# MaciejKozarzewski/AlphaGomoku

Hardware: AMD Instinct MI355X
Metric: MCTS simulations/sec (self-play, 15x15 freestyle) (higher is better)
Workload: dtype f16 (network, fp32 accumulate) + int/fp32 (tree)

## Files before the change

alphagomoku_amd/csrc/nn_forward.hip:

```cpp
#include "agx_internal.hpp"
#include "nn_any_board.hpp"

#include <vector>
#include <mutex>
#include <utility>
#include <cstring>
#include <cmath>
#include <cstdlib>
#include <type_traits>

#ifndef AGX_NN_COLS_AHEAD
#define AGX_NN_COLS_AHEAD 4
#endif
#ifndef AGX_NN_COLS_PAD
#define AGX_NN_COLS_PAD 1
#endif
#ifndef AGX_NN_ROW_GROUPS
#define AGX_NN_ROW_GROUPS 8
#endif
#ifndef AGX_NN_PAIR_BALANCE
#define AGX_NN_PAIR_BALANCE 1
#endif
#ifndef AGX_NN_AHEAD
#define AGX_NN_AHEAD 4
#endif

namespace
{
	typedef _Float16 half_t;
	typedef _Float16 half8 __attribute__((ext_vector_type(8)));
	typedef _Float16 half4 __attribute__((ext_vector_type(4)));
	typedef _Float16 half2 __attribute__((ext_vector_type(2)));
	typedef float floatx4 __attribute__((ext_vector_type(4)));

	struct NetParams
	{
			const half8 *w_in;
			const half8 *w_tower;
			const float *bias;
			const float *wp2;
			const float *wv1;
			const half_t *wv2;
			half_t *vhead_x;
			const float *bv2;
			const float *wv3;
			float bp2;
			float bv1[4];
			float bv3[3];
			int blocks;
			int batch;
			const int *slot_list;
			const int *count_ptr;
			const float *wq2;
			float bq2[3];
			float *q;
			half4 *skip;
	};

#ifdef AGX_NN_PROFILE
	__device__ unsigned long long g_nn_prof[2][16];
	struct NnStamp
	{
			unsigned long long last;
			bool on;
			int row;
			__device__ NnStamp(int wave, int lane) :
					last(clock64()), on(lane == 0 && (wave & 3) == 0), row(wave >> 2)
			{
			}
			__device__ void mark(int k)
			{
				const unsigned long long now = clock64();
				if (on)
					atomicAdd(&g_nn_prof[row][k], now - last);
				last = now;
			}
	};
#define AGX_NN_MARK(K) stamp.mark(K)
#define AGX_NN_STAMP_PARAM , NnStamp &stamp
#define AGX_NN_STAMP_ARG , stamp
#else
#define AGX_NN_MARK(K) do { } while (0)
#define AGX_NN_STAMP_PARAM
#define AGX_NN_STAMP_ARG
#endif

	template<int F, int ROWS, int COLS>
	struct Geometry
	{
			static constexpr int S = COLS + 1;
			static constexpr int NT = (ROWS * S + 15) / 16;
			static constexpr int NPOS = 1 + S + NT * 16 + S + 2;
			static constexpr int CH = F / 8;
			static constexpr int PPR = (16 / CH) > 0 ? (16 / CH) : 1;
			static constexpr bool COLT = (ROWS == 20 && COLS == 20 && F == 128);
			static constexpr int CG = (S == 16 && F >= 128) ? AGX_NN_ROW_GROUPS : ((S == 16 || F >= 128) ? 4 : 2);
			static constexpr int PG = 8 / CG;
			static constexpr int MT = F / (16 * CG);
			static constexpr int WRING = 2;
			static constexpr int STAGE_TAPS = 3;
			static constexpr int COL_TILES = COLS / PG, TAIL_TILES = 6 / PG, TAIL_FIRST = 21;
			static constexpr int PAD = COLT ? AGX_NN_COLS_PAD : 0;
			static constexpr int POS_BYTES = F * 2 + 16 * PAD;
			static constexpr int PLANE_BYTES = NPOS * POS_BYTES;
			static constexpr int NTW = COLT ? (COL_TILES + TAIL_TILES) : (NT + PG - 1) / PG;
			static constexpr int THREADS = 512;
			__device__ static __forceinline__ int channel_group(int wave) { return wave & (CG - 1); }
			__device__ static __forceinline__ int first_tile(int wave) { return (wave >> (CG == 8 ? 3 : (CG == 4 ? 2 : 1))) * NTW; }
			__device__ static __forceinline__ int swizzle(int index)
			{
				if constexpr (PAD > 0)
					return 0;
				else
					return (index / PPR) % CH;
			}
			__device__ static __forceinline__ int slot(int index, int chunk) { return chunk ^ swizzle(index); }
			__device__ static __forceinline__ int tile_position(int wave, int n, int r)
			{
				if constexpr (COLT)
				{
					const int pg = wave >> (CG == 8 ? 3 : 2);
					return (n < COL_TILES) ? (r * S + pg * COL_TILES + n) : ((TAIL_FIRST + pg * TAIL_TILES + (n - COL_TILES)) * 16 + r);
				}
				else
					return (first_tile(wave) + n) * 16 + r;
			}
			__device__ static __forceinline__ int tile_count(int wave)
			{
				if constexpr (COLT)
					return NTW;
				else if constexpr (PG == 1)
					return NT;
				else if constexpr (PG == 2)
					return (wave >> 2) ? (NT - NTW) : NTW;
				else
					return ((wave >> 1) == PG - 1) ? (NT - (PG - 1) * NTW) : NTW;
			}
			static constexpr int MTILES = F / 16;
			static constexpr int KC = F / 32;
			static constexpr int S5 = (S == 16 && F >= 128) ? 32 : S + 4;
			static constexpr int NPOS5 = (ROWS + 4) * S5 + 4;
			static constexpr int HW = ROWS * COLS;
			static constexpr int D = (2 * F < 256) ? 2 * F : 256;
			static constexpr int KPAD = (HW * 4 + 31) / 32 * 32;
			static constexpr int SCRATCH_FLOATS = HW * 4 + D + 8 + 256 + 8 + F * 4 + F + F * 4;
			static constexpr int LDS_BYTES = 2 * PLANE_BYTES + SCRATCH_FLOATS * 4;
			static constexpr int LDS_BYTES_INPLACE = PLANE_BYTES + SCRATCH_FLOATS * 4 + CG * NT * 16 * 4 + 3 * NT * 16 * 4;
			static constexpr int SKIP_PER_WG = 8 * MT * NTW * 64;
	};

	__device__ __forceinline__ void lds_barrier()
	{
		__builtin_amdgcn_fence(__ATOMIC_RELEASE, "workgroup", "local");
		__builtin_amdgcn_s_barrier();
		__builtin_amdgcn_fence(__ATOMIC_ACQUIRE, "workgroup", "local");
	}
	__device__ __forceinline__ int* pair_progress()
	{
		__shared__ int progress[8];
		return progress;
	}
	struct PairBalance
	{
			typedef __attribute__((address_space(3))) int lds_int;
			volatile lds_int *mine;
			const volatile lds_int *partner;
			int tick, seen;
			__device__ __forceinline__ PairBalance(int *progress, int wave) :
					mine((volatile lds_int*) (progress + wave)), partner((const volatile lds_int*) (progress + (wave ^ 4))), tick(progress[wave]), seen(progress[wave ^ 4])
			{
			}
			__device__ __forceinline__ void turn()
			{
#if AGX_NN_PAIR_BALANCE
				const int ahead = __builtin_amdgcn_readfirstlane(tick - seen);
				if (ahead > 0)
					__builtin_amdgcn_s_setprio(1);
				else if (ahead == 0)
					__builtin_amdgcn_s_setprio(2);
				else
					__builtin_amdgcn_s_setprio(3);
#endif
			}
			__device__ __forceinline__ void done()
			{
#if AGX_NN_PAIR_BALANCE
				tick++;
				*mine = tick;
				seen = *partner;
#endif
			}
	};
	template<typename G>
	__device__ __forceinline__ int plane_offset(int index, int chunk)
	{
		return index * G::POS_BYTES + G::slot(index, chunk) * 16;
// ... 924 lines not shown
						b[u] = fragment(u + 1);
#pragma unroll
					for (int j = 1; j <= G::NTW + 1; j++)
					{
						const int jn = j + AHEAD - 1;
						if (jn <= G::NTW + 1)
							b[(jn - 1) % AHEAD] = fragment(jn);
#pragma unroll
						for (int dyi = 3; dyi < 5; dyi++)
						{
							const int o = j - (dyi - 2);
							if (o >= 0 && o < G::NTW && o < my_tiles)
							{
#pragma unroll
								for (int i = 0; i < G::MT; i++)
									acc[i][o] = __builtin_amdgcn_mfma_f32_16x16x32_f16(a_down[dyi - 3][i], b[(j - 1) % AHEAD], acc[i][o], 0, 0, 0);
							}
						}
						__builtin_amdgcn_sched_barrier(0);
					}
				}
			}
		}
		else
		{
			int q0[G::NTW];
	#pragma unroll
			for (int n = 0; n < G::NTW; n++)
			{
				const int pos = G::S + G::tile_position(wave, n, r);
				const int x = pos % G::S;
				const int y = pos / G::S - 1;
				q0[n] = (y + 2) * G::S5 + (x + 2);
			}

			const half8 *wp = wpk + (mg * G::MT) * 64 + lane;
			half8 a_next[G::MT];
	#pragma unroll
			for (int i = 0; i < G::MT; i++)
				a_next[i] = wp[i * 64];
	#pragma unroll 1
			for (int t = 0; t < 25; t++)
			{
				const int off = (t / 5 - 2) * G::S5 + (t % 5 - 2);
				half8 a[G::MT];
	#pragma unroll
				for (int i = 0; i < G::MT; i++)
					a[i] = a_next[i];
				const int tn = (t + 1 < 25) ? (t + 1) : 0;
	#pragma unroll
				for (int i = 0; i < G::MT; i++)
					a_next[i] = wp[(tn * G::MTILES + i) * 64];
	#pragma unroll
				for (int n = 0; n < G::NTW; n++)
					if (n < my_tiles)
					{
						int q = q0[n] + off;
						q = (q < 0) ? 0 : ((q >= G::NPOS5) ? (G::NPOS5 - 1) : q);
						const half8 b = *reinterpret_cast<const half8*>(in5 + (q * 4 + (q4 ^ ((q >> 2) & 3))) * 16);
	#pragma unroll
						for (int i = 0; i < G::MT; i++)
							acc[i][n] = __builtin_amdgcn_mfma_f32_16x16x32_f16(a[i], b, acc[i][n], 0, 0, 0);
					}
			}
		}
		if (INPLACE)
		{
			__syncthreads();
			const uint4 zero4 = make_uint4(0u, 0u, 0u, 0u);
			for (int i = wave * 64 + lane; i < G::PLANE_BYTES / 16; i += G::THREADS)
				reinterpret_cast<uint4*>(dst)[i] = zero4;
			__syncthreads();
		}
		typedef __attribute__((address_space(1))) half4 global_half4;
		int skip_lane = lane;
		asm volatile("" : "+v"(skip_lane));
		global_half4 *my_skip = (global_half4*) (skip + __builtin_amdgcn_readfirstlane(wave * G::MT * G::NTW * 64)) + skip_lane;
		if constexpr (G::S == 16 && !INPLACE)
		{
			static_assert(G::NT == ROWS, "a tile is a board row + the spare column");
			if (r < COLS)
			{
#pragma unroll
				for (int i = 0; i < G::MT; i++)
				{
					const int ch = (mg * G::MT + i) * 16 + 4 * q4;
					const floatx4 bv = *reinterpret_cast<const floatx4*>(bias + ch);
					char *out0 = dst + plane_offset<G>(1 + G::S + n0 * 16 + r, ch / 8) + (ch % 8) * 2;
#pragma unroll
					for (int n = 0; n < G::NTW; n++)
						if (n < my_tiles)
						{
							const floatx4 v = acc[i][n];
							half2 lo { static_cast<half_t>(v[0] + bv[0]), static_cast<half_t>(v[1] + bv[1]) }, hi { static_cast<half_t>(v[2] + bv[2]), static_cast<half_t>(v[3] + bv[3]) };
							const half2 zero2 { static_cast<half_t>(0.0f), static_cast<half_t>(0.0f) };
							lo = __builtin_elementwise_max(lo, zero2);
							hi = __builtin_elementwise_max(hi, zero2);
							*reinterpret_cast<uint2*>(out0 + n * 16 * G::POS_BYTES) = uint2 { __builtin_bit_cast(uint32_t, lo), __builtin_bit_cast(uint32_t, hi) };
						}
				}
			}
			return;
		}
#pragma unroll
		for (int i = 0; i < G::MT; i++)
		{
			const int ch = (mg * G::MT + i) * 16 + 4 * q4;
			const floatx4 bv = *reinterpret_cast<const floatx4*>(bias + ch);
#pragma unroll
			for (int n = 0; n < G::NTW; n++)
				if (n < my_tiles)
				{
					const int pos = G::S + G::tile_position(wave, n, r);
					const int x = pos % G::S;
					const int y = pos / G::S - 1;
					const bool valid = (x < COLS) && (y < ROWS);
					char *ptr = dst + plane_offset<G>(pos + 1, ch / 8) + (ch % 8) * 2;
					const floatx4 v = acc[i][n] + bv;
					half4 o;
					o[0] = static_cast<half_t>(valid ? fmaxf(v[0], 0.0f) : 0.0f);
					o[1] = static_cast<half_t>(valid ? fmaxf(v[1], 0.0f) : 0.0f);
					o[2] = static_cast<half_t>(valid ? fmaxf(v[2], 0.0f) : 0.0f);
					o[3] = static_cast<half_t>(valid ? fmaxf(v[3], 0.0f) : 0.0f);
					*reinterpret_cast<half4*>(ptr) = o;
					if (INPLACE)
						my_skip[(i * G::NTW + n) * 64] = o;
				}
		}
	}

	__device__ __forceinline__ float block_reduce_max(float v, float *red, int tid)
	{
#pragma unroll
		for (int o = 32; o > 0; o >>= 1)
			v = fmaxf(v, __shfl_xor(v, o));
		__syncthreads();
		if ((tid & 63) == 0)
			red[tid >> 6] = v;
		__syncthreads();
		return fmaxf(fmaxf(fmaxf(red[0], red[1]), fmaxf(red[2], red[3])), fmaxf(fmaxf(red[4], red[5]), fmaxf(red[6], red[7])));
	}
	__device__ __forceinline__ float block_reduce_sum(float v, float *red, int tid)
	{
#pragma unroll
		for (int o = 32; o > 0; o >>= 1)
			v += __shfl_xor(v, o);
		__syncthreads();
		if ((tid & 63) == 0)
			red[tid >> 6] = v;
		__syncthreads();
		return ((red[0] + red[1]) + (red[2] + red[3])) + ((red[4] + red[5]) + (red[6] + red[7]));
	}

	template<int F, int ROWS, int COLS, bool INPLACE, bool QHEAD, bool RAW = false>
#ifndef AGX_NN_WAVES_PER_EU
#define AGX_NN_WAVES_PER_EU 2
#endif
	__global__ __launch_bounds__(256 * AGX_NN_WAVES_PER_EU) void nn_tower_kernel(NetParams p, const uint32_t *__restrict__ features, float *__restrict__ policy,
			float *__restrict__ value)
	{
		typedef Geometry<F, ROWS, COLS> G;
		constexpr int LDS_TOTAL = INPLACE ? G::LDS_BYTES_INPLACE : G::LDS_BYTES;
		static_assert(LDS_TOTAL <= 163840, "board does not fit in LDS");
		static_assert(G::NPOS5 * 64 <= G::PLANE_BYTES, "padded input plane must fit into an activation plane");
		__shared__ __attribute__((aligned(16))) char lds[LDS_TOTAL];
		char *plane_x = lds;
		char *plane_t = INPLACE ? lds : lds + G::PLANE_BYTES;
		float *vbuf = reinterpret_cast<float*>(lds + (INPLACE ? 1 : 2) * G::PLANE_BYTES);
		half8 *s_wv1f = reinterpret_cast<half8*>(vbuf);
		static_assert(G::KC * 64 * 16 <= (G::HW * 4 + G::D) * 4, "value-head fragments must fit into the former vbuf + hid area");
		float *hid = vbuf + G::HW * 4;
		float *red = hid + G::D;
		float *s_wv1 = red + 8 + 256 + 8;
		float *s_wp2 = s_wv1 + F * 4;
		float *s_wq2 = s_wp2 + F;
		float *ppart = s_wq2 + F * 4;
		float *qpart = ppart + G::CG * G::NT * 16;
		half4 *skip = INPLACE ? (p.skip + static_cast<size_t>(blockIdx.x) * G::SKIP_PER_WG) : nullptr;

		const int tid = threadIdx.x;
		const int wave = tid >> 6;
		const int lane = tid & 63;
		const int layer_halves8 = 9 * G::KC * G::MTILES * 64;

		const uint4 zero4 = make_uint4(0u, 0u, 0u, 0u);
		for (int i = tid; i < G::PLANE_BYTES / 16; i += G::THREADS)
			reinterpret_cast<uint4*>(plane_x)[i] = zero4;
		for (int i = tid; i < G::KC * 64; i += G::THREADS)
		{
			const int kc = i / 64, l = i % 64, unit = l & 15;
			half8 f;
#pragma unroll
			for (int j = 0; j < 8; j++)
				f[j] = static_cast<half_t>((unit < 4) ? p.wv1[(kc * 32 + 8 * (l >> 4) + j) * 4 + unit] : 0.0f);
			s_wv1f[i] = f;
		}
		for (int i = tid; i < F; i += G::THREADS)
			s_wp2[i] = p.wp2[i];
		if (QHEAD)
			for (int i = tid; i < F * 4; i += G::THREADS)
				s_wq2[i] = p.wq2[i];

#if AGX_NN_PAIR_BALANCE
		if (tid < 8)
			pair_progress()[tid] = 0;
#endif
		const int batch = (p.count_ptr != nullptr) ? min(*p.count_ptr, p.batch) : p.batch;
#ifdef AGX_NN_PROFILE
		NnStamp stamp(wave, lane);
#endif
		static_assert(G::HW <= G::THREADS, "one feature word per thread");
		uint32_t next_word = 0;
		if (static_cast<int>(blockIdx.x) < batch && tid < G::HW)
			next_word = features[static_cast<size_t>((p.slot_list != nullptr) ? p.slot_list[blockIdx.x] : static_cast<int>(blockIdx.x)) * G::HW + tid];
		for (int bi = blockIdx.x; bi < batch; bi += gridDim.x)
		{
			const int b = (p.slot_list != nullptr) ? p.slot_list[bi] : bi;
			__syncthreads();
			for (int i = tid; i < G::NPOS5 * (RAW ? 1 : 4); i += G::THREADS)
				reinterpret_cast<uint4*>(plane_t)[i] = zero4;
			__syncthreads();
			for (int c = tid; c < G::HW; c += G::THREADS)
			{
				const uint32_t word = next_word;
				const int q = (c / COLS + 2) * G::S5 + (c % COLS + 2);
#pragma unroll
				for (int k = 0; k < (RAW ? 1 : 4); k++)
				{
					const uint32_t bits = (word >> (8 * k)) & 255u;
					uint4 v;
					v.x = ((bits & 1u) ? 0x3C00u : 0u) | ((bits & 2u) ? 0x3C000000u : 0u);
					v.y = ((bits & 4u) ? 0x3C00u : 0u) | ((bits & 8u) ? 0x3C000000u : 0u);
					v.z = ((bits & 16u) ? 0x3C00u : 0u) | ((bits & 32u) ? 0x3C000000u : 0u);
					v.w = ((bits & 64u) ? 0x3C00u : 0u) | ((bits & 128u) ? 0x3C000000u : 0u);
					if (RAW)
						*reinterpret_cast<uint4*>(plane_t + q * 16) = v;
					else
						*reinterpret_cast<uint4*>(plane_t + (q * 4 + (k ^ ((q >> 2) & 3))) * 16) = v;
				}
			}
			__syncthreads();
			AGX_NN_MARK(0);
			conv5x5_input<F, ROWS, COLS, INPLACE, RAW>(plane_t, plane_x, p.w_in, p.bias, skip, wave, lane);
			BiasCarry<G::MT> bias_carry;
			request_bias<G>(p.bias + F, wave, lane, bias_carry);
			__syncthreads();
			AGX_NN_MARK(1);
			if (!INPLACE)
			{
				for (int i = tid; i < G::PLANE_BYTES / 16; i += G::THREADS)
					reinterpret_cast<uint4*>(plane_t)[i] = zero4;
				__syncthreads();
			}

			AGX_NN_MARK(9);
			constexpr bool CARRY = INPLACE ? (G::COLT && !RAW) : G::S == 16;
			WeightCarry<G> carry_store;
			WeightCarry<G> *carry = CARRY ? &carry_store : nullptr;
			if constexpr (CARRY)
				request_first_stage<F, ROWS, COLS>(p.w_tower, wave, lane, carry_store);
			for (int blk = 0; blk < p.blocks; blk++)
			{
				if (INPLACE)
				{
					SkipCarry<G> skip_carry;
					if constexpr (CARRY)
						carry_store.next = p.w_tower + (2 * blk + 1) * layer_halves8;
					conv3x3_inplace<F, ROWS, COLS, 0>(plane_x, p.w_tower + (2 * blk) * layer_halves8, bias_carry, p.bias + (2 + 2 * blk) * F, skip, nullptr, nullptr, wave,
							lane AGX_NN_STAMP_ARG, &skip_carry, carry);
					lds_barrier();
					if constexpr (CARRY)
						carry_store.next = p.w_tower + (2 * blk + 2) * layer_halves8;
					conv3x3_inplace<F, ROWS, COLS, 1>(plane_x, p.w_tower + (2 * blk + 1) * layer_halves8, bias_carry, p.bias + (3 + 2 * blk) * F, skip, nullptr, nullptr, wave,
							lane AGX_NN_STAMP_ARG, &skip_carry, carry);
					lds_barrier();
				}
				else
				{
					if constexpr (CARRY)
						carry_store.next = p.w_tower + (2 * blk + 1) * layer_halves8;
					conv3x3<F, ROWS, COLS, false>(plane_x, plane_t, p.w_tower + (2 * blk) * layer_halves8, p.bias + (1 + 2 * blk) * F, wave, lane AGX_NN_STAMP_ARG, carry, &bias_carry,
							p.bias + (2 + 2 * blk) * F);
					__syncthreads();
					AGX_NN_MARK(5);
					if constexpr (CARRY)
						carry_store.next = p.w_tower + (2 * blk + 2) * layer_halves8;
					conv3x3<F, ROWS, COLS, true>(plane_t, plane_x, p.w_tower + (2 * blk + 1) * layer_halves8, p.bias + (2 + 2 * blk) * F, wave, lane AGX_NN_STAMP_ARG, carry, &bias_carry,
							p.bias + (3 + 2 * blk) * F);
					__syncthreads();
					AGX_NN_MARK(5);
				}
			}

			{
				const int r = lane & 15, q4 = lane >> 4;
				for (int n = wave; n < G::NT; n += G::THREADS / 64)
				{
					floatx4 v { p.bv1[0], p.bv1[1], p.bv1[2], p.bv1[3] };
					const int index0 = 1 + G::S + n * 16 + r;
#pragma unroll
					for (int kc = 0; kc < G::KC; kc++)
					{
						const half8 bfrag = *reinterpret_cast<const half8*>(plane_x + plane_offset<G>(index0, kc * 4 + q4));
						v = __builtin_amdgcn_mfma_f32_16x16x32_f16(s_wv1f[kc * 64 + lane], bfrag, v, 0, 0, 0);
					}
					const int pos = G::S + n * 16 + r;
					const int x = pos % G::S, y = pos / G::S - 1;
					if (q4 == 0 && x < COLS && y < ROWS)
					{
						half4 o;
						o[0] = static_cast<half_t>(fmaxf(v[0], 0.0f));
						o[1] = static_cast<half_t>(fmaxf(v[1], 0.0f));
						o[2] = static_cast<half_t>(fmaxf(v[2], 0.0f));
						o[3] = static_cast<half_t>(fmaxf(v[3], 0.0f));
						*reinterpret_cast<half4*>(p.vhead_x + static_cast<size_t>(bi) * G::KPAD + (y * COLS + x) * 4) = o;
					}
				}
			}
			AGX_NN_MARK(6);
			if (INPLACE)
			{
				if constexpr (CARRY)
					carry_store.next = p.w_tower + (2 * p.blocks) * layer_halves8;
				conv3x3_inplace<F, ROWS, COLS, 2>(plane_x, p.w_tower + (2 * p.blocks) * layer_halves8, bias_carry, QHEAD ? p.bias + (2 + 2 * p.blocks) * F : nullptr, nullptr, s_wp2,
						ppart, wave, lane AGX_NN_STAMP_ARG, nullptr, carry);
			}
			else
			{
				if constexpr (CARRY)
					carry_store.next = p.w_tower + (2 * p.blocks) * layer_halves8;
				conv3x3<F, ROWS, COLS, false>(plane_x, plane_t, p.w_tower + (2 * p.blocks) * layer_halves8, p.bias + (1 + 2 * p.blocks) * F, wave, lane AGX_NN_STAMP_ARG, carry,
						&bias_carry, p.bias + (1 + 2 * p.blocks) * F);
			}
			__syncthreads();
			AGX_NN_MARK(7);
			if (bi + static_cast<int>(gridDim.x) < batch && tid < G::HW)
			{
				const int nb = bi + static_cast<int>(gridDim.x);
				next_word = features[static_cast<size_t>((p.slot_list != nullptr) ? p.slot_list[nb] : nb) * G::HW + tid];
			}

			{
				float logit = -3.0e38f;
				const int c = tid;
				if (c < G::HW)
				{
					float s = p.bp2;
					if (INPLACE)
					{
						const int idx = (c / COLS) * G::S + (c % COLS);
						constexpr int PS = G::NT * 16;
						if constexpr (G::CG == 8)
							s += ((ppart[idx] + ppart[PS + idx]) + (ppart[2 * PS + idx] + ppart[3 * PS + idx]))
									+ ((ppart[4 * PS + idx] + ppart[5 * PS + idx]) + (ppart[6 * PS + idx] + ppart[7 * PS + idx]));
						else if constexpr (G::CG == 4)
							s += (ppart[idx] + ppart[PS + idx]) + (ppart[2 * PS + idx] + ppart[3 * PS + idx]);
						else
							s += ppart[idx] + ppart[PS + idx];
					}
					else
					{
						const int index = 1 + G::S + (c / COLS) * G::S + (c % COLS);
						for (int k = 0; k < G::CH; k++)
						{
							const half8 tv = *reinterpret_cast<const half8*>(plane_t + plane_offset<G>(index, k));
#pragma unroll
							for (int j = 0; j < 8; j++)
								s += static_cast<float>(tv[j]) * s_wp2[k * 8 + j];
						}
					}
					logit = s;
				}
				static_assert(G::HW <= G::THREADS, "policy softmax assumes one cell per thread");
				const float m = block_reduce_max(logit, red, tid);
				const float e = (c < G::HW) ? __expf(logit - m) : 0.0f;
				const float sum = block_reduce_sum(e, red, tid);
				if (c < G::HW)
					policy[static_cast<size_t>(b) * G::HW + c] = e / sum;
			}

			if (QHEAD)
			{
				const half8 *wq1 = p.w_tower + (2 * p.blocks + 1) * layer_halves8;
				const float *bq1 = p.bias + (2 + 2 * p.blocks) * F;
				__syncthreads();
				if (INPLACE)
					conv3x3_inplace<F, ROWS, COLS, 3>(plane_x, wq1, bias_carry, nullptr, nullptr, s_wq2, qpart, wave, lane AGX_NN_STAMP_ARG);
				else
				{
					conv3x3<F, ROWS, COLS, false, true>(plane_x, plane_t, wq1, bq1, wave, lane AGX_NN_STAMP_ARG);
					__syncthreads();
				}
				const int c = tid;
				if (c < G::HW)
				{
					float z0 = p.bq2[0], z1 = p.bq2[1], z2 = p.bq2[2];
					if (INPLACE)
					{
						const int idx = (c / COLS) * G::S + (c % COLS);
						z0 += qpart[idx];
						z1 += qpart[G::NT * 16 + idx];
						z2 += qpart[2 * G::NT * 16 + idx];
					}
					else
					{
						const int index = 1 + G::S + (c / COLS) * G::S + (c % COLS);
						for (int k = 0; k < G::CH; k++)
						{
							const half8 tv = *reinterpret_cast<const half8*>(plane_t + plane_offset<G>(index, k));
#pragma unroll
							for (int j = 0; j < 8; j++)
							{
								const float t = static_cast<float>(tv[j]);
								const floatx4 w = *reinterpret_cast<const floatx4*>(s_wq2 + (k * 8 + j) * 4);
								z0 += t * w[0];
								z1 += t * w[1];
								z2 += t * w[2];
							}
						}
					}
					const float m = fmaxf(z0, fmaxf(z1, z2));
					const float e0 = __expf(z0 - m), e1 = __expf(z1 - m), e2 = __expf(z2 - m);
					const float inv = 1.0f / (e0 + e1 + e2);
					float *out = p.q + (static_cast<size_t>(b) * G::HW + c) * 2;
					out[0] = e0 * inv;
					out[1] = e1 * inv;
				}
			}
			AGX_NN_MARK(8);
		}
	}

	template<int KPAD, int D>
	__global__ __launch_bounds__(256) void value_head_kernel(const half_t *__restrict__ x, const half8 *__restrict__ w2, const float *__restrict__ b2,
			const float *__restrict__ w3, float b30, float b31, float b32, const int *__restrict__ slot_list, const int *__restrict__ count_ptr, int batch_cap,
			float *__restrict__ value)
	{
		constexpr int MTW = D / 64;
		__shared__ float hid[16][D + 1];
		const int batch = (count_ptr != nullptr) ? min(*count_ptr, batch_cap) : batch_cap;
		const int b0 = blockIdx.x * 16;
		if (b0 >= batch)
			return;
		const int tid = threadIdx.x, wave = tid >> 6, lane = tid & 63, r = lane & 15, q4 = lane >> 4;
		const int board = min(b0 + r, batch - 1);
		floatx4 acc[MTW];
#pragma unroll
		for (int i = 0; i < MTW; i++)
			acc[i] = floatx4 { 0.0f, 0.0f, 0.0f, 0.0f };
		const half8 *xb = reinterpret_cast<const half8*>(x + static_cast<size_t>(board) * KPAD) + q4;
		const half8 *wp = w2 + (wave * MTW) * 64 + lane;
#pragma unroll 4
		for (int kc = 0; kc < KPAD / 32; kc++)
		{
			const half8 bfrag = xb[kc * 4];
#pragma unroll
			for (int i = 0; i < MTW; i++)
				acc[i] = __builtin_amdgcn_mfma_f32_16x16x32_f16(wp[(kc * (D / 16) + i) * 64], bfrag, acc[i], 0, 0, 0);
		}
#pragma unroll
		for (int i = 0; i < MTW; i++)
		{
			const int u = (wave * MTW + i) * 16 + 4 * q4;
#pragma unroll
			for (int e = 0; e < 4; e++)
				hid[r][u + e] = fmaxf(acc[i][e] + b2[u + e], 0.0f);
		}
		__syncthreads();
		__shared__ float logits[16][3];
		if (tid < 48)
		{
			const int bb = tid / 3, o = tid % 3;
			float sacc = 0.0f;
			for (int j = 0; j < D; j++)
				sacc += hid[bb][j] * w3[j * 3 + o];
			logits[bb][o] = sacc + ((o == 0) ? b30 : ((o == 1) ? b31 : b32));
		}
		__syncthreads();
		if (tid < 16 && b0 + tid < batch)
		{
			const int bi = b0 + tid;
			const int slot = (slot_list != nullptr) ? slot_list[bi] : bi;
			const float z0 = logits[tid][0], z1 = logits[tid][1], z2 = logits[tid][2];
			const float m = fmaxf(z0, fmaxf(z1, z2));
			const float e0 = __expf(z0 - m), e1 = __expf(z1 - m), e2 = __expf(z2 - m);
			const float inv = 1.0f / (e0 + e1 + e2);
			value[static_cast<size_t>(slot) * 3 + 0] = e0 * inv;
			value[static_cast<size_t>(slot) * 3 + 1] = e1 * inv;
			value[static_cast<size_t>(slot) * 3 + 2] = e2 * inv;
		}
	}

	void pack_conv(const float *w, int taps, int cin, int cout, std::vector<half_t> &dst)
	{
		const int kcs = cin / 32;
		const int mtiles = cout / 16;
		const size_t base = dst.size();
		dst.resize(base + static_cast<size_t>(taps) * kcs * mtiles * 512);
		half_t *out = dst.data() + base;
		for (int t = 0; t < taps; t++)
			for (int kc = 0; kc < kcs; kc++)
				for (int mt = 0; mt < mtiles; mt++)
					for (int lane = 0; lane < 64; lane++)
						for (int j = 0; j < 8; j++)
						{
							const int oc = mt * 16 + (lane & 15);
							const int ic = kc * 32 + 8 * (lane >> 4) + j;
							const float v = w[(static_cast<size_t>(t) * cin + ic) * cout + oc];
							out[(((static_cast<size_t>(t) * kcs + kc) * mtiles + mt) * 64 + lane) * 8 + j] = static_cast<half_t>(v);
						}
	}
}

namespace
{
	void pack_conv_rows(const float *w, int cin, int cout, std::vector<half_t> &dst, bool by_row_shift = false, int groups = 4)
	{
		const int kcs = cin / 32, mt_per_group = cout / (16 * groups);
		const size_t base = dst.size();
		dst.resize(base + static_cast<size_t>(9) * kcs * (cout / 16) * 512);
		half_t *out = dst.data() + base;
		size_t frag = 0;
		for (int kc = 0; kc < kcs; kc++)
			for (int dx = 0; dx < 3; dx++)
				for (int mg = 0; mg < groups; mg++)
					for (int dy = 0; dy < 3; dy++)
						for (int i = 0; i < mt_per_group; i++, frag++)
							for (int lane = 0; lane < 64; lane++)
								for (int j = 0; j < 8; j++)
								{
									const int t = by_row_shift ? (dx * 3 + dy) : (dy * 3 + dx);
									const int oc = (mg * mt_per_group + i) * 16 + (lane & 15);
									const int ic = kc * 32 + 8 * (lane >> 4) + j;
									out[(frag * 64 + lane) * 8 + j] = static_cast<half_t>(w[(static_cast<size_t>(t) * cin + ic) * cout + oc]);
								}
	}
}

namespace
{
	void pack_conv5x5_raw(const float *w, int cout, std::vector<half_t> &dst)
	{
		const int mtiles = cout / 16;
		dst.assign(static_cast<size_t>(10) * mtiles * 512, static_cast<half_t>(0.0f));
		for (int t = 0; t < 10; t++)
			for (int mt = 0; mt < mtiles; mt++)
				for (int lane = 0; lane < 64; lane++)
				{
					const int dy = t / 2, dx = 4 * (t % 2) + (lane >> 4);
					if (dx >= 5)
						continue;
					for (int j = 0; j < 8; j++)
						dst[((static_cast<size_t>(t) * mtiles + mt) * 64 + lane) * 8 + j] = static_cast<half_t>(w[(static_cast<size_t>(dy * 5 + dx) * 8 + j) * cout + mt * 16 + (lane & 15)]);
				}
	}
}

struct AgxNet
{
		AgxNetDesc desc;
		bool loaded = false;
		void *d_w_in = nullptr;
		void *d_w_tower = nullptr;
		void *d_bias = nullptr;
		void *d_wp2 = nullptr;
		void *d_wv1 = nullptr;
		void *d_wv2 = nullptr;
		void *d_bv2 = nullptr;
		void *d_wv3 = nullptr;
		void *d_wq2 = nullptr;
		float bq2[3] = { 0, 0, 0 };
		std::mutex skip_mutex;
		struct StreamScratch
		{
				hipStream_t stream;
				void *skip;
				void *vhead;
				int vhead_boards;
		};
		std::vector<StreamScratch> scratch_by_stream;
		size_t skip_bytes = 0;
		bool inplace = false;
		bool any_board = false;
		float bp2 = 0.0f;
		float bv1[4] = { 0, 0, 0, 0 };
		float bv3[3] = { 0, 0, 0 };
		int num_cus = 256;
		int launch_width = 0;
};

namespace
{
	bool is_supported(const AgxNetDesc &d)
	{
		return d.rows >= agx_any::MIN_SIDE && d.rows <= agx_any::MAX_SIDE && d.cols >= agx_any::MIN_SIDE && d.cols <= agx_any::MAX_SIDE && (d.filters == 64 || d.filters == 128) && d.blocks >= 0
				&& (d.in_channels == 32 || (d.in_channels == 8 && d.action_values == 0))
				&& d.value_hidden == ((2 * d.filters < 256) ? 2 * d.filters : 256) && (d.action_values == 0 || d.action_values == 1);
	}
	void free_net_buffers(AgxNet *net)
	{
		void **ptrs[] = { &net->d_w_in, &net->d_w_tower, &net->d_bias, &net->d_wp2, &net->d_wv1, &net->d_wv2, &net->d_bv2, &net->d_wv3, &net->d_wq2 };
		for (void **p : ptrs)
		{
			if (*p != nullptr)
				(void) hipFree(*p);
			*p = nullptr;
		}
		std::lock_guard<std::mutex> lock(net->skip_mutex);
		for (auto &slice : net->scratch_by_stream)
		{
			if (slice.skip != nullptr)
				(void) hipFree(slice.skip);
			if (slice.vhead != nullptr)
				(void) hipFree(slice.vhead);
		}
		net->scratch_by_stream.clear();
	}
	template<typename T>
	int upload(void **dst, const std::vector<T> &src)
	{
		AGX_HIP_CHECK(hipMalloc(dst, src.size() * sizeof(T)));
		AGX_HIP_CHECK(hipMemcpy(*dst, src.data(), src.size() * sizeof(T), hipMemcpyHostToDevice));
		return AGX_OK;
	}
}

extern "C" {

size_t agx_net_blob_floats(const AgxNetDesc *d)
{
	if (d == nullptr)
		return 0;
	const size_t F = d->filters, C = d->in_channels, HW = static_cast<size_t>(d->rows) * d->cols, D = d->value_hidden;
	size_t n = 25 * C * F + F;
	n += static_cast<size_t>(d->blocks) * 2 * (9 * F * F + F);
	n += 9 * F * F + F + F + 1;
	n += F * 4 + 4 + HW * 4 * D + D + D * 3 + 3;
	if (d->action_values)
		n += 9 * F * F + F + F * 3 + 3;
	return n;
}

int agx_net_create(const AgxNetDesc *desc, AgxNet **out)
{
	AGX_REQUIRE(desc != nullptr && out != nullptr, AGX_ERR_INVALID, "agx_net_create: null argument");
	AGX_REQUIRE(is_supported(*desc), AGX_ERR_UNSUPPORTED,
			"agx_net_create: unsupported network %dx%d blocks=%d filters=%d cin=%d hidden=%d (supported: 5..20 rows and cols, F in {64,128}, cin 32, or cin 8 without the action-values head)", desc->rows,
			desc->cols, desc->blocks, desc->filters, desc->in_channels, desc->value_hidden);
	AgxNet *net = new AgxNet();
	net->desc = *desc;
	int dev = 0;
	hipDeviceProp_t prop;
	if (hipGetDevice(&dev) == hipSuccess && hipGetDeviceProperties(&prop, dev) == hipSuccess)
		net->num_cus = prop.multiProcessorCount;
	*out = net;
	return AGX_OK;
}

int agx_net_load_weights(AgxNet *net, const float *h_blob, size_t n_floats)
{
	AGX_REQUIRE(net != nullptr && h_blob != nullptr, AGX_ERR_INVALID, "agx_net_load_weights: null argument");
	AGX_REQUIRE(n_floats == agx_net_blob_floats(&net->desc), AGX_ERR_INVALID, "agx_net_load_weights: blob has %zu floats, expected %zu", n_floats,
			agx_net_blob_floats(&net->desc));
	free_net_buffers(net);
	net->loaded = false;

	const int F = net->desc.filters, C = net->desc.in_channels, HW = net->desc.rows * net->desc.cols, D = net->desc.value_hidden;
	const int blocks = net->desc.blocks;
	const float *ptr = h_blob;

	std::vector<half_t> w_in, w_tower, wv2;
	std::vector<float> bias, wp2, wv1, bv2, wv3;

	if (C == 8)
		pack_conv5x5_raw(ptr, F, w_in);
	else
		pack_conv(ptr, 25, C, F, w_in);
	ptr += 25 * C * F;
	bias.insert(bias.end(), ptr, ptr + F);
	ptr += F;
	const bool board15 = (net->desc.rows == 15 && net->desc.cols == 15), board20 = (net->desc.rows == 20 && net->desc.cols == 20);
	const char *any = getenv("AGX_NN_ANY_BOARD");
	net->any_board = !(board15 || board20) || (any != nullptr && any[0] == '1');
	const bool row_order = board15 && !net->any_board;
	const bool column_order = board20 && F == 128 && !net->any_board;
	auto pack3x3 = [&](const float *w)
	{
		if (row_order)
			pack_conv_rows(w, F, F, w_tower, false, (F == 128) ? Geometry<128, 15, 15>::CG : Geometry<64, 15, 15>::CG);
		else if (column_order)
			pack_conv_rows(w, F, F, w_tower, true, Geometry<128, 20, 20>::CG);
		else
			pack_conv(w, 9, F, F, w_tower);
	};
	for (int l = 0; l < 2 * blocks + 1; l++)
	{
		pack3x3(ptr);
		ptr += 9 * F * F;
		bias.insert(bias.end(), ptr, ptr + F);
		ptr += F;
	}
	wp2.assign(ptr, ptr + F);
	ptr += F;
	net->bp2 = *ptr++;
	wv1.assign(ptr, ptr + F * 4);
	ptr += F * 4;
	for (int i = 0; i < 4; i++)
		net->bv1[i] = *ptr++;
	{
		const int kpad = (HW * 4 + 31) / 32 * 32, mtiles = D / 16;
		wv2.assign(static_cast<size_t>(kpad) * D, static_cast<half_t>(0.0f));
		for (int kc = 0; kc < kpad / 32; kc++)
			for (int mt = 0; mt < mtiles; mt++)
				for (int lane = 0; lane < 64; lane++)
					for (int j = 0; j < 8; j++)
					{
						const int unit = mt * 16 + (lane & 15), k = kc * 32 + 8 * (lane >> 4) + j;
						if (k < HW * 4)
							wv2[((static_cast<size_t>(kc) * mtiles + mt) * 64 + lane) * 8 + j] = static_cast<half_t>(ptr[static_cast<size_t>(k) * D + unit]);
					}
	}
	ptr += static_cast<size_t>(HW) * 4 * D;
	bv2.assign(ptr, ptr + D);
	ptr += D;
	wv3.assign(ptr, ptr + D * 3);
	ptr += D * 3;
	for (int i = 0; i < 3; i++)
		net->bv3[i] = *ptr++;
	std::vector<float> wq2;
	if (net->desc.action_values)
	{
		pack3x3(ptr);
		ptr += 9 * F * F;
		bias.insert(bias.end(), ptr, ptr + F);
		ptr += F;
		wq2.assign(static_cast<size_t>(F) * 4, 0.0f);
		for (int c = 0; c < F; c++)
			for (int o = 0; o < 3; o++)
				wq2[c * 4 + o] = ptr[c * 3 + o];
		ptr += F * 3;
		for (int i = 0; i < 3; i++)
			net->bq2[i] = *ptr++;
	}

	const char *force = getenv("AGX_NN_SINGLE_PLANE");
	net->inplace = net->any_board || board20 || (force != nullptr && force[0] == '1');
	if (net->any_board)
		net->skip_bytes = agx_any::skip_bytes_per_workgroup(F) * static_cast<size_t>(net->num_cus);
	else if (net->inplace)
	{
		const size_t per_wg = board20 ? ((F == 128) ? Geometry<128, 20, 20>::SKIP_PER_WG : Geometry<64, 20, 20>::SKIP_PER_WG)
				: ((F == 128) ? Geometry<128, 15, 15>::SKIP_PER_WG : Geometry<64, 15, 15>::SKIP_PER_WG);
		net->skip_bytes = per_wg * 8 * static_cast<size_t>(net->num_cus);
	}
	int status = AGX_OK;
	if ((status = upload(&net->d_w_in, w_in)) != AGX_OK || (status = upload(&net->d_w_tower, w_tower)) != AGX_OK
			|| (status = upload(&net->d_bias, bias)) != AGX_OK || (status = upload(&net->d_wp2, wp2)) != AGX_OK
			|| (status = upload(&net->d_wv1, wv1)) != AGX_OK || (status = upload(&net->d_wv2, wv2)) != AGX_OK
			|| (status = upload(&net->d_bv2, bv2)) != AGX_OK || (status = upload(&net->d_wv3, wv3)) != AGX_OK
			|| (!wq2.empty() && (status = upload(&net->d_wq2, wq2)) != AGX_OK))
	{
		free_net_buffers(net);
		return status;
	}
	net->loaded = true;
	return AGX_OK;
}

static int launch_forward(AgxNet *net, const uint32_t *d_features, const int *d_slot_list, const int *d_count, int batch, float *d_policy, float *d_value,
		float *d_action_values, void *stream)
{
	AGX_REQUIRE(net != nullptr, AGX_ERR_INVALID, "agx_nn_forward: null network");
	AGX_REQUIRE(net->loaded, AGX_ERR_STATE, "agx_nn_forward: weights not loaded");
	AGX_REQUIRE(batch >= 0, AGX_ERR_INVALID, "agx_nn_forward: negative batch");
	if (batch == 0)
		return AGX_OK;
	AGX_REQUIRE(d_features != nullptr && d_policy != nullptr && d_value != nullptr, AGX_ERR_INVALID, "agx_nn_forward: null buffer");

	NetParams p;
	p.w_in = static_cast<const half8*>(net->d_w_in);
	p.w_tower = static_cast<const half8*>(net->d_w_tower);
	p.bias = static_cast<const float*>(net->d_bias);
	p.wp2 = static_cast<const float*>(net->d_wp2);
	p.wv1 = static_cast<const float*>(net->d_wv1);
	p.wv2 = static_cast<const half_t*>(net->d_wv2);
	p.bv2 = static_cast<const float*>(net->d_bv2);
	p.wv3 = static_cast<const float*>(net->d_wv3);
	p.bp2 = net->bp2;
	for (int i = 0; i < 4; i++)
		p.bv1[i] = net->bv1[i];
	for (int i = 0; i < 3; i++)
		p.bv3[i] = net->bv3[i];
	p.blocks = net->desc.blocks;
	p.batch = batch;
	p.slot_list = d_slot_list;
	p.count_ptr = d_count;
	AGX_REQUIRE(d_action_values == nullptr || net->desc.action_values, AGX_ERR_INVALID, "agx_nn_forward: the network has no action-values head");
	p.q = d_action_values;
	p.wq2 = (d_action_values != nullptr) ? static_cast<const float*>(net->d_wq2) : nullptr;
	for (int i = 0; i < 3; i++)
		p.bq2[i] = net->bq2[i];

	const int width = (net->launch_width > 0 && net->launch_width < net->num_cus) ? net->launch_width : net->num_cus;
	const int grid = (batch < width) ? batch : width;
	hipStream_t s = static_cast<hipStream_t>(stream);
	p.skip = nullptr;
	const int kpad = (net->desc.rows * net->desc.cols * 4 + 31) / 32 * 32;
	{
		std::lock_guard<std::mutex> lock(net->skip_mutex);
		AgxNet::StreamScratch *mine = nullptr;
		for (auto &slice : net->scratch_by_stream)
			if (slice.stream == s)
				mine = &slice;
		if (mine == nullptr)
		{
			net->scratch_by_stream.push_back(AgxNet::StreamScratch { s, nullptr, nullptr, 0 });
			mine = &net->scratch_by_stream.back();
		}
		if (net->inplace && mine->skip == nullptr)
			AGX_HIP_CHECK(hipMalloc(&mine->skip, net->skip_bytes));
		if (mine->vhead_boards < batch)
		{
			if (mine->vhead != nullptr)
			{
				AGX_HIP_CHECK(hipStreamSynchronize(s));
				AGX_HIP_CHECK(hipFree(mine->vhead));
				mine->vhead = nullptr;
			}
			const size_t bytes = static_cast<size_t>(batch) * kpad * sizeof(half_t);
			AGX_HIP_CHECK(hipMalloc(&mine->vhead, bytes));
			AGX_HIP_CHECK(hipMemsetAsync(mine->vhead, 0, bytes, s));
			mine->vhead_boards = batch;
		}
		p.skip = static_cast<half4*>(mine->skip);
		p.vhead_x = static_cast<half_t*>(mine->vhead);
	}
	if (net->any_board)
	{
		agx_any::Params a;
		a.w_in = p.w_in;
		a.w_tower = p.w_tower;
		a.bias = p.bias;
		a.wp2 = p.wp2;
		a.wv1 = p.wv1;
		a.wv2 = p.wv2;
		a.vhead_x = p.vhead_x;
		a.bv2 = p.bv2;
		a.wv3 = p.wv3;
		a.bp2 = p.bp2;
		for (int i = 0; i < 4; i++)
			a.bv1[i] = p.bv1[i];
		for (int i = 0; i < 3; i++)
		{
			a.bv3[i] = p.bv3[i];
			a.bq2[i] = p.bq2[i];
		}
		a.blocks = p.blocks;
		a.batch = p.batch;
		a.slot_list = p.slot_list;
		a.count_ptr = p.count_ptr;
		a.wq2 = p.wq2;
		a.q = p.q;
		a.skip = p.skip;
		a.rows = net->desc.rows;
		a.cols = net->desc.cols;
		return agx_any::launch(a, net->desc.filters, net->desc.in_channels == 8, grid, d_features, d_policy, d_value, s);
	}
	const bool big = (net->desc.rows == 20 && net->desc.cols == 20), wide = (net->desc.filters == 128), qhead = (p.q != nullptr), raw = (net->desc.in_channels == 8);
	const dim3 g(grid), t(512);
#define AGX_LAUNCH_TOWER(FF, NN, IP, QH, RW) hipLaunchKernelGGL((nn_tower_kernel<FF, NN, NN, IP, QH, RW>), g, t, 0, s, p, d_features, d_policy, d_value)
#define AGX_LAUNCH_HEADS(FF, NN, IP) do { if (qhead) AGX_LAUNCH_TOWER(FF, NN, IP, true, false); else if (raw) AGX_LAUNCH_TOWER(FF, NN, IP, false, true); \
		else AGX_LAUNCH_TOWER(FF, NN, IP, false, false); } while (0)
	if (net->inplace)
	{
		if (big && wide)
			AGX_LAUNCH_HEADS(128, 20, true);
		else if (big)
			AGX_LAUNCH_HEADS(64, 20, true);
		else if (wide)
			AGX_LAUNCH_HEADS(128, 15, true);
		else
			AGX_LAUNCH_HEADS(64, 15, true);
	}
	else if (wide)
		AGX_LAUNCH_HEADS(128, 15, false);
	else
		AGX_LAUNCH_HEADS(64, 15, false);
#undef AGX_LAUNCH_HEADS
#undef AGX_LAUNCH_TOWER
	{
		const dim3 vg((batch + 15) / 16), vt(256);
#define AGX_LAUNCH_VALUE(KP, DD) hipLaunchKernelGGL((value_head_kernel<KP, DD>), vg, vt, 0, s, p.vhead_x, reinterpret_cast<const half8*>(p.wv2), p.bv2, p.wv3, \
		p.bv3[0], p.bv3[1], p.bv3[2], d_slot_list, d_count, batch, d_value)
		if (big && wide)
			AGX_LAUNCH_VALUE(1600, 256);
		else if (big)
			AGX_LAUNCH_VALUE(1600, 128);
		else if (wide)
			AGX_LAUNCH_VALUE(928, 256);
		else
			AGX_LAUNCH_VALUE(928, 128);
#undef AGX_LAUNCH_VALUE
	}
	AGX_HIP_CHECK(hipGetLastError());
	return AGX_OK;
}

int agx_nn_forward(AgxNet *net, const uint32_t *d_features, int batch, float *d_policy, float *d_value, void *stream)
{
	return launch_forward(net, d_features, nullptr, nullptr, batch, d_policy, d_value, nullptr, stream);
}
int agx_nn_forward_pvq(AgxNet *net, const uint32_t *d_features, int batch, float *d_policy, float *d_value, float *d_action_values, void *stream)
{
	return launch_forward(net, d_features, nullptr, nullptr, batch, d_policy, d_value, d_action_values, stream);
}
int agx_nn_forward_indirect(AgxNet *net, const uint32_t *d_features, const int *d_slot_list, const int *d_count, int max_batch, float *d_policy,
		float *d_value, void *stream)
{
	AGX_REQUIRE(d_slot_list != nullptr && d_count != nullptr, AGX_ERR_INVALID, "agx_nn_forward_indirect: null list");
	return launch_forward(net, d_features, d_slot_list, d_count, max_batch, d_policy, d_value, nullptr, stream);
}
int agx_nn_forward_indirect_pvq(AgxNet *net, const uint32_t *d_features, const int *d_slot_list, const int *d_count, int max_batch, float *d_policy,
		float *d_value, float *d_action_values, void *stream)
{
	AGX_REQUIRE(d_slot_list != nullptr && d_count != nullptr, AGX_ERR_INVALID, "agx_nn_forward_indirect_pvq: null list");
	return launch_forward(net, d_features, d_slot_list, d_count, max_batch, d_policy, d_value, d_action_values, stream);
}

#ifdef AGX_NN_PROFILE
int agx_debug_nn_profile(unsigned long long *out)
{
	AGX_HIP_CHECK(hipDeviceSynchronize());
	AGX_HIP_CHECK(hipMemcpyFromSymbol(out, HIP_SYMBOL(g_nn_prof), sizeof(unsigned long long) * 32));
	unsigned long long zero[32] = { 0 };
	AGX_HIP_CHECK(hipMemcpyToSymbol(HIP_SYMBOL(g_nn_prof), zero, sizeof(zero)));
	return AGX_OK;
}
#endif

int agx_net_set_launch_width(AgxNet *net, int workgroups)
{
	AGX_REQUIRE(net != nullptr && workgroups >= 0, AGX_ERR_INVALID, "agx_net_set_launch_width: invalid argument");
	net->launch_width = workgroups;
	return AGX_OK;
}

int agx_net_description(const AgxNet *net, AgxNetDesc *out)
{
	AGX_REQUIRE(net != nullptr && out != nullptr, AGX_ERR_INVALID, "agx_net_description: null argument");
	*out = net->desc;
	return AGX_OK;
}

int agx_net_destroy(AgxNet *net)
{
	if (net == nullptr)
		return AGX_OK;
	free_net_buffers(net);
	delete net;
	return AGX_OK;
}

}
```

Measured before the change: 1.030 million.

## Fuse value-head dense layers into tower kernel via per-tile arrival counters

Each workgroup now atomically stores its value-head conv output and bumps a per-16-board counter. The last workgroup to arrive for a tile computes that tile's dense value head inside the tower kernel. This removes the separate value_head_kernel launch and its dependency gap. The cost is atomics, an acquire fence and serialized tail work on whichever workgroup finishes last. The old path stays available through an environment variable.

```diff
diff --git a/alphagomoku_amd/csrc/nn_forward.hip b/alphagomoku_amd/csrc/nn_forward.hip
--- a/alphagomoku_amd/csrc/nn_forward.hip
+++ b/alphagomoku_amd/csrc/nn_forward.hip
@@ -32,6 +32,8 @@
 	typedef _Float16 half4 __attribute__((ext_vector_type(4)));
 	typedef _Float16 half2 __attribute__((ext_vector_type(2)));
 	typedef float floatx4 __attribute__((ext_vector_type(4)));
+	typedef __attribute__((address_space(1))) unsigned long long global_u64;
+	typedef __attribute__((address_space(1))) int global_int;
 
 	struct NetParams
 	{
@@ -42,6 +44,7 @@
 			const float *wv1;
 			const half_t *wv2;
 			half_t *vhead_x;
+			int *vcount;
 			const float *bv2;
 			const float *wv3;
 			float bp2;
@@ -1272,6 +1275,67 @@
 		return ((red[0] + red[1]) + (red[2] + red[3])) + ((red[4] + red[5]) + (red[6] + red[7]));
 	}
 
+	template<int KPAD, int D, int WAVES>
+	__device__ __forceinline__ void value_head_tile(const half_t *x, const half8 *w2, const float *b2, const float *w3, float b30, float b31, float b32,
+			const int *slot_list, int batch, int b0, float (*hid)[D + 1], float (*logits)[3], float *value, int tid)
+	{
+		constexpr int MTW = D / (16 * WAVES);
+		static_assert(MTW >= 1 && MTW * 16 * WAVES == D, "the hidden units are whole tiles per wave");
+		const int wave = tid >> 6, lane = tid & 63, r = lane & 15, q4 = lane >> 4;
+		const int board = min(b0 + r, batch - 1);
+		floatx4 acc[MTW];
+#pragma unroll
+		for (int i = 0; i < MTW; i++)
+			acc[i] = floatx4 { 0.0f, 0.0f, 0.0f, 0.0f };
+		const half8 *xb = reinterpret_cast<const half8*>(x + static_cast<size_t>(board) * KPAD) + q4;
+		const half8 *wp = w2 + (wave * MTW) * 64 + lane;
+#pragma unroll 4
+		for (int kc = 0; kc < KPAD / 32; kc++)
+		{
+			const half8 bfrag = xb[kc * 4];
+#pragma unroll
+			for (int i = 0; i < MTW; i++)
+				acc[i] = __builtin_amdgcn_mfma_f32_16x16x32_f16(wp[(kc * (D / 16) + i) * 64], bfrag, acc[i], 0, 0, 0);
+		}
+#pragma unroll
+		for (int i = 0; i < MTW; i++)
+		{
+			const int u = (wave * MTW + i) * 16 + 4 * q4;
+#pragma unroll
+			for (int e = 0; e < 4; e++)
+				hid[r][u + e] = fmaxf(acc[i][e] + b2[u + e], 0.0f);
+		}
+		__syncthreads();
+		if (tid < 48)
+		{
+			const int bb = tid / 3, o = tid % 3;
+			float sacc = 0.0f;
+			for (int j = 0; j < D; j++)
+				sacc += hid[bb][j] * w3[j * 3 + o];
+			logits[bb][o] = sacc + ((o == 0) ? b30 : ((o == 1) ? b31 : b32));
+		}
+		__syncthreads();
+		if (tid < 16 && b0 + tid < batch)
+		{
+			const int bi = b0 + tid;
+			const int slot = (slot_list != nullptr) ? slot_list[bi] : bi;
+			const float z0 = logits[tid][0], z1 = logits[tid][1], z2 = logits[tid][2];
+			const float m = fmaxf(z0, fmaxf(z1, z2));
+			const float e0 = __expf(z0 - m), e1 = __expf(z1 - m), e2 = __expf(z2 - m);
+			const float inv = 1.0f / (e0 + e1 + e2);
+			value[static_cast<size_t>(slot) * 3 + 0] = e0 * inv;
+			value[static_cast<size_t>(slot) * 3 + 1] = e1 * inv;
+			value[static_cast<size_t>(slot) * 3 + 2] = e2 * inv;
+		}
+	}
+
+	template<int KPAD, int D, int WAVES>
+	__device__ __attribute__((noinline)) void value_head_tile_call(const half_t *x, const half8 *w2, const float *b2, const float *w3, float b30, float b31, float b32,
+			const int *slot_list, int batch, int b0, float (*hid)[D + 1], float (*logits)[3], float *value, int tid)
+	{
+		value_head_tile<KPAD, D, WAVES>(x, w2, b2, w3, b30, b31, b32, slot_list, batch, b0, hid, logits, value, tid);
+	}
+
 	template<int F, int ROWS, int COLS, bool INPLACE, bool QHEAD, bool RAW = false>
 #ifndef AGX_NN_WAVES_PER_EU
 #define AGX_NN_WAVES_PER_EU 2
@@ -1291,6 +1355,7 @@
 		static_assert(G::KC * 64 * 16 <= (G::HW * 4 + G::D) * 4, "value-head fragments must fit into the former vbuf + hid area");
 		float *hid = vbuf + G::HW * 4;
 		float *red = hid + G::D;
+		int *tile_flag = reinterpret_cast<int*>(red + 8);
 		float *s_wv1 = red + 8 + 256 + 8;
 		float *s_wp2 = s_wv1 + F * 4;
 		float *s_wq2 = s_wp2 + F;
@@ -1433,7 +1498,8 @@
 						o[1] = static_cast<half_t>(fmaxf(v[1], 0.0f));
 						o[2] = static_cast<half_t>(fmaxf(v[2], 0.0f));
 						o[3] = static_cast<half_t>(fmaxf(v[3], 0.0f));
-						*reinterpret_cast<half4*>(p.vhead_x + static_cast<size_t>(bi) * G::KPAD + (y * COLS + x) * 4) = o;
+						__hip_atomic_store((global_u64*) (p.vhead_x + static_cast<size_t>(bi) * G::KPAD + (y * COLS + x) * 4), __builtin_bit_cast(unsigned long long, o),
+								__ATOMIC_RELAXED, __HIP_MEMORY_SCOPE_AGENT);
 					}
 				}
 			}
@@ -1454,6 +1520,9 @@
 			}
 			__syncthreads();
 			AGX_NN_MARK(7);
+			int ticket = -1;
+			if (p.vcount != nullptr && tid == 0)
+				ticket = __hip_atomic_fetch_add((global_int*) (p.vcount + (bi >> 4)), 1, __ATOMIC_RELAXED, __HIP_MEMORY_SCOPE_AGENT);
 			if (bi + static_cast<int>(gridDim.x) < batch && tid < G::HW)
 			{
 				const int nb = bi + static_cast<int>(gridDim.x);
@@ -1494,6 +1563,14 @@
 				static_assert(G::HW <= G::THREADS, "policy softmax assumes one cell per thread");
 				const float m = block_reduce_max(logit, red, tid);
 				const float e = (c < G::HW) ? __expf(logit - m) : 0.0f;
+				if (tid == 0)
+				{
+					const int need = min(16, batch - (bi & ~15));
+					const bool last = (ticket == need - 1);
+					if (last)
+						__hip_atomic_store((global_int*) (p.vcount + (bi >> 4)), 0, __ATOMIC_RELAXED, __HIP_MEMORY_SCOPE_AGENT);
+					*tile_flag = last ? 1 : 0;
+				}
 				const float sum = block_reduce_sum(e, red, tid);
 				if (c < G::HW)
 					policy[static_cast<size_t>(b) * G::HW + c] = e / sum;
@@ -1547,6 +1624,20 @@
 					out[1] = e1 * inv;
 				}
 			}
+			if (__builtin_amdgcn_readfirstlane(*tile_flag) != 0)
+			{
+				if (tid == 0)
+				{
+					__builtin_amdgcn_fence(__ATOMIC_ACQUIRE, "agent");
+					asm volatile("s_waitcnt vmcnt(0)" ::: "memory");
+				}
+				__syncthreads();
+				static_assert((16 * (G::D + 1) + 48) * 4 <= G::PLANE_BYTES, "hid and the logits must fit into the plane");
+				float (*tile_hid)[G::D + 1] = reinterpret_cast<float (*)[G::D + 1]>(plane_t);
+				float (*tile_logits)[3] = reinterpret_cast<float (*)[3]>(plane_t + 16 * (G::D + 1) * 4);
+				value_head_tile_call<G::KPAD, G::D, G::THREADS / 64>(p.vhead_x, reinterpret_cast<const half8*>(p.wv2), p.bv2, p.wv3, p.bv3[0], p.bv3[1], p.bv3[2], p.slot_list, batch,
+						bi & ~15, tile_hid, tile_logits, value, tid);
+			}
 			AGX_NN_MARK(8);
 		}
 	}
@@ -1556,59 +1647,13 @@
 			const float *__restrict__ w3, float b30, float b31, float b32, const int *__restrict__ slot_list, const int *__restrict__ count_ptr, int batch_cap,
 			float *__restrict__ value)
 	{
-		constexpr int MTW = D / 64;
 		__shared__ float hid[16][D + 1];
+		__shared__ float logits[16][3];
 		const int batch = (count_ptr != nullptr) ? min(*count_ptr, batch_cap) : batch_cap;
 		const int b0 = blockIdx.x * 16;
 		if (b0 >= batch)
 			return;
-		const int tid = threadIdx.x, wave = tid >> 6, lane = tid & 63, r = lane & 15, q4 = lane >> 4;
-		const int board = min(b0 + r, batch - 1);
-		floatx4 acc[MTW];
-#pragma unroll
-		for (int i = 0; i < MTW; i++)
-			acc[i] = floatx4 { 0.0f, 0.0f, 0.0f, 0.0f };
-		const half8 *xb = reinterpret_cast<const half8*>(x + static_cast<size_t>(board) * KPAD) + q4;
-		const half8 *wp = w2 + (wave * MTW) * 64 + lane;
-#pragma unroll 4
-		for (int kc = 0; kc < KPAD / 32; kc++)
-		{
-			const half8 bfrag = xb[kc * 4];
-#pragma unroll
-			for (int i = 0; i < MTW; i++)
-				acc[i] = __builtin_amdgcn_mfma_f32_16x16x32_f16(wp[(kc * (D / 16) + i) * 64], bfrag, acc[i], 0, 0, 0);
-		}
-#pragma unroll
-		for (int i = 0; i < MTW; i++)
-		{
-			const int u = (wave * MTW + i) * 16 + 4 * q4;
-#pragma unroll
-			for (int e = 0; e < 4; e++)
-				hid[r][u + e] = fmaxf(acc[i][e] + b2[u + e], 0.0f);
-		}
-		__syncthreads();
-		__shared__ float logits[16][3];
-		if (tid < 48)
-		{
-			const int bb = tid / 3, o = tid % 3;
-			float sacc = 0.0f;
-			for (int j = 0; j < D; j++)
-				sacc += hid[bb][j] * w3[j * 3 + o];
-			logits[bb][o] = sacc + ((o == 0) ? b30 : ((o == 1) ? b31 : b32));
-		}
-		__syncthreads();
-		if (tid < 16 && b0 + tid < batch)
-		{
-			const int bi = b0 + tid;
-			const int slot = (slot_list != nullptr) ? slot_list[bi] : bi;
-			const float z0 = logits[tid][0], z1 = logits[tid][1], z2 = logits[tid][2];
-			const float m = fmaxf(z0, fmaxf(z1, z2));
-			const float e0 = __expf(z0 - m), e1 = __expf(z1 - m), e2 = __expf(z2 - m);
-			const float inv = 1.0f / (e0 + e1 + e2);
-			value[static_cast<size_t>(slot) * 3 + 0] = e0 * inv;
-			value[static_cast<size_t>(slot) * 3 + 1] = e1 * inv;
-			value[static_cast<size_t>(slot) * 3 + 2] = e2 * inv;
-		}
+		value_head_tile<KPAD, D, 4>(x, w2, b2, w3, b30, b31, b32, slot_list, batch, b0, hid, logits, value, threadIdx.x);
 	}
 
 	void pack_conv(const float *w, int taps, int cin, int cout, std::vector<half_t> &dst)
@@ -1697,10 +1742,12 @@
 				void *skip;
 				void *vhead;
 				int vhead_boards;
+				void *vcount;
 		};
 		std::vector<StreamScratch> scratch_by_stream;
 		size_t skip_bytes = 0;
 		bool inplace = false;
+		bool separate_value_head = false;
 		bool any_board = false;
 		float bp2 = 0.0f;
 		float bv1[4] = { 0, 0, 0, 0 };
@@ -1733,6 +1780,8 @@
 				(void) hipFree(slice.skip);
 			if (slice.vhead != nullptr)
 				(void) hipFree(slice.vhead);
+			if (slice.vcount != nullptr)
+				(void) hipFree(slice.vcount);
 		}
 		net->scratch_by_stream.clear();
 	}
@@ -1865,6 +1914,8 @@
 
 	const char *force = getenv("AGX_NN_SINGLE_PLANE");
 	net->inplace = net->any_board || board20 || (force != nullptr && force[0] == '1');
+	const char *separate = getenv("AGX_NN_SEPARATE_VALUE_HEAD");
+	net->separate_value_head = (separate != nullptr && separate[0] == '1');
 	if (net->any_board)
 		net->skip_bytes = agx_any::skip_bytes_per_workgroup(F) * static_cast<size_t>(net->num_cus);
 	else if (net->inplace)
@@ -1934,7 +1985,7 @@
 				mine = &slice;
 		if (mine == nullptr)
 		{
-			net->scratch_by_stream.push_back(AgxNet::StreamScratch { s, nullptr, nullptr, 0 });
+			net->scratch_by_stream.push_back(AgxNet::StreamScratch { s, nullptr, nullptr, 0, nullptr });
 			mine = &net->scratch_by_stream.back();
 		}
 		if (net->inplace && mine->skip == nullptr)
@@ -1946,14 +1997,20 @@
 				AGX_HIP_CHECK(hipStreamSynchronize(s));
 				AGX_HIP_CHECK(hipFree(mine->vhead));
 				mine->vhead = nullptr;
+				AGX_HIP_CHECK(hipFree(mine->vcount));
+				mine->vcount = nullptr;
 			}
 			const size_t bytes = static_cast<size_t>(batch) * kpad * sizeof(half_t);
 			AGX_HIP_CHECK(hipMalloc(&mine->vhead, bytes));
 			AGX_HIP_CHECK(hipMemsetAsync(mine->vhead, 0, bytes, s));
+			const size_t counter_bytes = (static_cast<size_t>((batch + 15) / 16) * sizeof(int) + 15) / 16 * 16;
+			AGX_HIP_CHECK(hipMalloc(&mine->vcount, counter_bytes));
+			AGX_HIP_CHECK(hipMemsetAsync(mine->vcount, 0, counter_bytes, s));
 			mine->vhead_boards = batch;
 		}
 		p.skip = static_cast<half4*>(mine->skip);
 		p.vhead_x = static_cast<half_t*>(mine->vhead);
+		p.vcount = (net->separate_value_head || net->any_board) ? nullptr : static_cast<int*>(mine->vcount);
 	}
 	if (net->any_board)
 	{
@@ -2008,6 +2065,7 @@
 		AGX_LAUNCH_HEADS(64, 15, false);
 #undef AGX_LAUNCH_HEADS
 #undef AGX_LAUNCH_TOWER
+	if (p.vcount == nullptr)
 	{
 		const dim3 vg((batch + 15) / 16), vt(256);
 #define AGX_LAUNCH_VALUE(KP, DD) hipLaunchKernelGGL((value_head_kernel<KP, DD>), vg, vt, 0, s, p.vhead_x, reinterpret_cast<const half8*>(p.wv2), p.bv2, p.wv3, \
```

Measured after the change: 937,700. -8.9%, worse.
